# Xinglab/abPOA

Measured on AMD Instinct MI355X. Metric: read-sets/sec (consensus bit-exact) + DP Gcells/sec (roofline.dp_gcells_per_s), higher is better.
Workload: dtype int16

## Files before the change

### abpoa_amd/csrc/engine.cpp

```cpp
#include <hip/hip_runtime.h>
#include <stdio.h>
#include <stdlib.h>
#include <string.h>
#include <stdarg.h>
#include <limits.h>
#include <mutex>
#include <vector>
#include <algorithm>
#include "engine_options.h"
#include "batch_stream.h"
#include "routing.h"
#include "dir_plane.h"

namespace abpoa_hip {

static char g_err[512] = ""; static std::mutex g_err_mu;
static thread_local char g_err_copy[512] = "";
static thread_local char tl_err[512] = "";
void set_err(const char *fmt, ...) {
    va_list ap; va_start(ap, fmt); vsnprintf(tl_err, sizeof(tl_err), fmt, ap); va_end(ap);
    std::lock_guard<std::mutex> lk(g_err_mu);
    memcpy(g_err, tl_err, sizeof(g_err));
}
const char *thread_last_error() { return tl_err; }
void clear_thread_error() { tl_err[0] = 0; }
#define HIP_TRY(expr, code)                                                                          \
    do { hipError_t e_ = (expr); if (e_ != hipSuccess) {                                             \
// ... 351 lines not shown
const char *abpoa_hip_last_error(void) { std::lock_guard<std::mutex> lk(g_err_mu); memcpy(g_err_copy, g_err, sizeof(g_err)); return g_err_copy; }
void abpoa_hip_get_stats(abpoa_hip_stats_t *out) { std::lock_guard<std::mutex> lk(g.stats_mu); *out = g.stats; }
void abpoa_hip__dir_counts(long long *out) { out[0] = __atomic_exchange_n(&g_dir_counts[0], 0, __ATOMIC_RELAXED); out[1] = __atomic_exchange_n(&g_dir_counts[1], 0, __ATOMIC_RELAXED); }
void abpoa_hip__wide_plan(const abpoa_hip_scoring_t *sc, int max_qlen, int max_bits, int n_aln, int *out) {
    abpoa_hip::LdsPlan L; const int pn = max_bits == 16 ? 16 : 8; const int w = sc->wb + (int)(sc->wf * (float)max_qlen);
    abpoa_hip::make_lds_plan(sc, max_qlen, max_bits, abpoa_hip::band_cols(abpoa_hip::padded_width(max_qlen, pn), w, pn, true), n_aln, &L);
    out[0] = L.wide_on; out[1] = L.wfr_rows; out[2] = L.total_wide; out[3] = L.total_wide > 0 ? abpoa_hip::wide_workgroups_per_cu(L.total_wide) : 0;
    out[4] = L.w_phase_off; out[5] = L.wide_w_lo; out[6] = L.wide_w_hi;
}
void abpoa_hip__narrow_plan(const abpoa_hip_scoring_t *sc, int max_qlen, int max_bits, int n_aln, int *out) {
    abpoa_hip::LdsPlan L; const int pn = max_bits == 16 ? 16 : 8; const int w = sc->wb + (int)(sc->wf * (float)max_qlen);
    abpoa_hip::make_lds_plan(sc, max_qlen, max_bits, abpoa_hip::band_cols(abpoa_hip::padded_width(max_qlen, pn), w, pn, true), n_aln, &L);
    out[0] = L.fr_rows; out[1] = L.fr_cols; out[2] = L.bt_bytes_tail;
}
void abpoa_hip__row_launches(long long *out) { for (int i = 0; i < 3; ++i) out[i] = __atomic_exchange_n(&abpoa_hip::g_row_launches[i], 0, __ATOMIC_RELAXED); }
void abpoa_hip__debug_clocks(long long *out) { for (int i = 0; i < 10; ++i) { out[i] = g_dbg[i]; g_dbg[i] = 0; } }
void abpoa_hip_reset_stats(void) { std::lock_guard<std::mutex> lk(g.stats_mu); memset(&g.stats, 0, sizeof(g.stats)); }

void abpoa_hip_free_result(abpoa_hip_result_t *r) {
    if (!r) return;
    free(r->cigar);
    if (r->trace) {
        abpoa_hip_trace_t *t = r->trace;
        free(t->dp_beg); free(t->dp_end); free(t->dp_beg_sn); free(t->dp_end_sn); free(t->row_off); free(t->planes); free(t->row_max_i); free(t);
    }
    memset(r, 0, sizeof(*r));
}

static int validate(const abpoa_hip_scoring_t *sc, const abpoa_hip_problem_t *p, int idx) {
    if (p->n_rows < 3 || p->qlen < 0) { set_err("problem %d: n_rows=%d qlen=%d", idx, p->n_rows, p->qlen); return ABPOA_HIP_EINVAL; }
// ... 75 lines not shown
```

### abpoa_amd/csrc/engine_options.cpp

```cpp
#include "engine_options.h"
#include <atomic>
#include <cstdlib>
#include <cstring>
#include <mutex>
#include <string>

namespace abpoa_hip {
namespace {

struct Row { const char *name, *help; };
const Row kTable[] = {
    {"ABPOA_GPU_DEVICES", "P  device ordinals abpoa_hip_msa_batch spreads its batches over: all | 0,1,... (default: the device of abpoa_hip_init)"},
    {"ABPOA_GPU_BATCHES_PER_DEVICE", "P  batches dealt per device queue [2]"},
    {"ABPOA_HIP_STRICT", "P  1: a call that would hand any read-set to the host driver fails with ABPOA_HIP_ESTRICT"},
    {"ABPOA_HIP_VERBOSE", "P  per-pass timings, residency and fallback reasons on stderr"},
    {"ABPOA_HIP_HOSTGRAPH", "T  1: the host driver for every job"},
    {"ABPOA_HIP_NO_DEVICE_STRAND", "T  1: -s jobs on the host driver"},
    {"ABPOA_HIP_NO_DEVICE_LOCAL", "T  1: local-mode jobs on the host driver"},
    {"ABPOA_HIP_NO_DEVICE_GENERAL", "T  1: general-kernel jobs on the host driver"},
    {"ABPOA_HIP_DEVICE_GENERAL", "T  1: the general kernel for every device-resident job"},
    {"ABPOA_HIP_LOCKSTEP", "T  1: one launch per phase and round also where the all-rounds kernel would run"},
    {"ABPOA_HIP_LATE_TAIL", "T  1: the helpers of the all-rounds kernel's backtrack start after the row loop, not under it"},
    {"ABPOA_HIP_NODIR", "T  1: score-record arenas instead of direction words"},
    {"ABPOA_HIP_DIR_WIDE", "T  1 / 0: direction words for wide-band alignments always / never (default: by residency and memory)"},
    {"ABPOA_HIP_NOFAST", "T  1: no fast row loops (general kernel)"},
    {"ABPOA_HIP_NOWIDE", "T  1: no wide row loop"},
    {"ABPOA_HIP_NOXL", "T  1: no long-read form of the wide row loop"},
    {"ABPOA_HIP_LOCAL_TEAM", "T  1 / 0: the four-wavefront local row loop always / never"},
    {"ABPOA_HIP_WIDE_LO", "T  smallest band half-width that takes the wide loop [40]"},
    {"ABPOA_HIP_RING_ROWS", "T  depth of the wide loop's score ring (4 | 8 | 16)"},
    {"ABPOA_HIP_EXTRA_ROUTE_MIN", "T  ragged sets with fewer extra columns keep the narrow loop"},
    {"ABPOA_HIP_NO_RAGGED_SPLIT", "T  1: read-sets with ragged read ends stay in the batch of the uniform ones (no all-rounds kernel for such a job)"},
    {"ABPOA_HIP_RAGGED_CONCURRENT", "T  1: the ragged batch of a mixed job runs on a second queue of the device beside the uniform batch (measured: see LOG.md)"},
    {"ABPOA_HIP_PASS_SETS", "T  read-sets per pass of the device-resident driver"},
    {"ABPOA_HIP_FIRST_PASS", "T  start the node-slot ladder (3x, 4.5x, 6x, 4096x) at its second / third / fourth pass: 1 / 2 / 3 (profiling runs of one step)"},
    {"ABPOA_HIP_NO_PASS_HINT", "T  1: always start the ladder at 3x"},
    {"ABPOA_HIP_GROUPS", "T  read-set groups of the host driver"},
// ... 64 lines not shown
```

### abpoa_amd/csrc/msa_batch.cpp

```cpp
#include <algorithm>
#include <atomic>
#include <stdio.h>
#include <chrono>
#include <condition_variable>
#include <functional>
#include <memory>
#include <mutex>
#include <stdlib.h>
#include <string.h>
#include <thread>
#include <vector>
#include "engine_options.h"
#include "msa_batch.h"
#include "poa_graph.h"

#include <unordered_map>
namespace abpoa_hip {

namespace {
std::mutex g_dig_mu; std::unordered_map<uint64_t, uint64_t> g_dig;
uint64_t digest_mix64(uint64_t z) { z += 0x9E3779B97F4A7C15ull; z = (z ^ (z >> 30)) * 0xBF58476D1CE4E5B9ull; z = (z ^ (z >> 27)) * 0x94D049BB133111EBull; return z ^ (z >> 31); }
uint64_t digest_word_mix(uint64_t word, int i) { return digest_mix64(word + 0xD6E8FEB86659FD93ull * (uint64_t)(i + 1)); }
uint64_t digest_round(uint64_t before, int read_index, int n_cigar, uint64_t sum) { return (before * 0x9E3779B97F4A7C15ull) ^ (sum + digest_mix64(((uint64_t)(uint32_t)read_index
        << 32) | (uint32_t)n_cigar)); }
// ... 156 lines not shown
            if (rc) return rc;
            t2 = now_s();
            pool.run((int)active.size(), [&](int a) {
                const int s = active[a];
                if (fwd_st[a] != 0) { out[s].status = fwd_st[a]; return; }
                out[s].n_cells += fwd_cells[a];
                const uint64_t *cg = fwd_cig[a].data(); int ncg = (int)fwd_cig[a].size();
                const uint8_t *q = sets[s].seqs[k]; const int32_t *wq = weights_of(sets[s], k);
                const auto it = std::find(retry.begin(), retry.end(), a);
                if (it != retry.end()) {
                    const int t = (int)(it - retry.begin());
                    if (al->status(t) != 0) { out[s].status = al->status(t); return; }
                    out[s].n_cells += al->n_cells(t);
                    if (al->best_score(t) > fwd_score[a]) { cg = al->cigar(t); ncg = al->n_cigar(t); q = rc_seq[a].data(); wq = wq ? rc_w[a].data() : nullptr; if (out[s].is_rc) out[s].is_rc[k] = 1; }
                }
                try { graphs[s].add_alignment(q, sets[s].lens[k], cg, ncg, k, wq); } catch (...) { fail.store(1); }
            });
        } else
        pool.run((int)active.size(), [&](int a) {
            const int s = active[a];
            const int st = al->status(a);
            if (st != 0) { out[s].status = st; return; }
            out[s].n_cells += al->n_cells(a);
            if (cigar_digest_on()) cigar_digest_add(sets[s].seqs[0], sets[s].lens[0], k, al->cigar(a), al->n_cigar(a));
            try { graphs[s].add_alignment(sets[s].seqs[k], sets[s].lens[k], al->cigar(a), al->n_cigar(a), k, weights_of(sets[s], k)); } catch (...) { fail.store(1); }
        });
        if (fail.load()) return ABPOA_HIP_EINVAL;
        const double t3 = now_s();
        gt->sort_s += t1 - t0; gt->engine_s += t2 - t1; gt->fuse_s += t3 - t2; gt->rounds += 1;
    }
// ... 111 lines not shown
```

### abpoa_amd/csrc/msa_device.cpp

```cpp
#include <algorithm>
#include <atomic>
#include <chrono>
#include <limits.h>
#include <mutex>
#include <stdio.h>
#include <stdlib.h>
#include <string.h>
#include <thread>
#include <vector>
#include <hip/hip_runtime.h>
#include "engine_options.h"
#include "batch_stream.h"
#include "msa_device.h"
#include "poa_device.h"
#include "poa_graph.h"
#include "dir_plane.h"
#include "msa_batch.h"
#include "msa_device_debug.h"
#include "msa_device_plan.h"
#include "routing.h"

namespace abpoa_hip {

namespace {
#define HIP_OK(expr, code) do { hipError_t e_ = (expr); if (e_ != hipSuccess) { \
        set_err("%s failed: %s (%s:%d)", #expr, hipGetErrorString(e_), __FILE__, __LINE__); return code; } } while (0)

double now_s() { return std::chrono::duration<double>(std::chrono::steady_clock::now().time_since_epoch()).count(); }

template <typename F>
void parallel_ranges(int n_threads, int n, F fn) {
    const int T = std::max(1, std::min(n_threads, n / 64));
    if (T <= 1) { fn(0, n); return; }
    std::vector<std::thread> th; th.reserve(T - 1);
    for (int t = 0; t < T - 1; ++t) th.emplace_back(fn, (int)((int64_t)n * t / T), (int)((int64_t)n * (t + 1) / T));
// ... 45 lines not shown
    size_t o_cnode, o_ccov, o_cbase, o_isrc;
    size_t o_state, o_base, o_nin, o_nout, o_naln, o_in, o_out, o_outw, o_inx, o_outx, o_outwx, o_aln, o_nread, o_row, o_order0, o_order1, o_rid, o_mrank,
            o_msaoff, o_tout, o_toutw, o_tin, graph_bytes;
    size_t o_ticket, o_aln_desc, o_out_rec, o_rbase, o_rsd, o_rpd, o_rnid, o_rrem, o_poff, o_pred, o_bsn, o_esn, o_coff, o_rmi, o_cigar, o_scratch, o_ooff,
            o_orow, o_left, o_right, o_act, o_outfwd, o_cigfwd, o_retry, rows_bytes;
};

struct Job {
    DevicePlan pl; const abpoa_hip_readset_t *sets; int n_sets, n_threads, device, slot;
    Cache *C; Layout L; size_t dl_bytes;
    bool any_w, rest_up; int64_t split_at;
    PoaDev p; DevBatch b, b_rc, b_r;
    bool dbg_sync, use_rounds; size_t rounds_lds;
    std::vector<int64_t> msa_off;
    double t_begin, t_queue, t_done;
};

}

void release_msa_device_caches() {
    int cur = -1; (void)hipGetDevice(&cur);
    for (int s = 0; s < MSA_DEVICE_SLOTS; ++s) {
        std::lock_guard<std::mutex> lk(g_cache_mu[s]);
        Cache &C = g_cache[s];
        if (C.device < 0) continue;
        (void)hipSetDevice(C.device);
        if (C.stream) (void)hipStreamSynchronize(C.stream);
        C.release();
    }
    if (cur >= 0) (void)hipSetDevice(cur);
}

// ... 77 lines not shown
    if (need > free_b + given_back) {
        if (opt_set("ABPOA_HIP_VERBOSE")) fprintf(stderr,
                "[abpoa-hip] device %d: %d sets need %.1f GB in growing buffers (arenas %.1f GB), %.1f GB free + %.1f " "GB given back: splitting\n",
                J.device, J.n_sets, need / 1e9, pl.plane_tot / 1e9, free_b / 1e9, given_back / 1e9);
        set_err("device-resident job needs %zu more bytes, %zu free", need, free_b + given_back); return ABPOA_HIP_ENOMEM;
    }
    int rc;
    if ((rc = C.in.need_dev(L.in_dev_bytes)) || (rc = C.in.need_host(L.in_bytes)) || (rc = C.graph.need_dev(L.graph_bytes)) || (rc =
            C.graph.need_host(J.dl_bytes)) ||
        (rc = C.rows.need_dev(L.rows_bytes)) || (rc = C.planes.need_dev((size_t)pl.plane_tot))) return rc;
    const int n_ev = 4 * pl.max_reads + 8;
    while ((int)C.ev.size() < n_ev) { hipEvent_t e; HIP_OK(hipEventCreate(&e), ABPOA_HIP_ENODEV); C.ev.push_back(e); }
    return 0;
}

void stage_reads(const Job &J, int k_lo, int k_hi) {
    const DevicePlan &pl = J.pl; uint8_t *hi = J.C->in.host; const int64_t *roff = (const int64_t *)(hi + J.L.o_roff); uint8_t *rd = hi + J.L.o_reads;
    parallel_ranges(std::min(J.n_threads, 16), J.n_sets, [&](int lo, int hi_) {
        for (int s = lo; s < hi_; ++s) { const int64_t r0 = pl.ps[s].read0; const int ke = std::min(k_hi, J.sets[s].n_reads);
                for (int r = k_lo; r < ke; ++r) memcpy(rd + roff[r0 + r], J.sets[s].seqs[r], J.sets[s].lens[r]); }
    });
}

int upload_reads(Job &J) {
    const DevicePlan &pl = J.pl; Cache &C = *J.C; const Layout &L = J.L; const abpoa_hip_scoring_t *sc = &pl.sc;
    uint8_t *hi = C.in.host;
    memcpy(hi + L.o_sets, pl.ps.data(), sizeof(PoaSet) * J.n_sets);
    int64_t *roff = (int64_t *)(hi + L.o_roff); int32_t *rlen = (int32_t *)(hi + L.o_rlen); uint8_t *rd = hi + L.o_reads;
    J.split_at = 0;
    {
        int64_t at = 0;
        for (int k = 0; k < pl.max_reads; ++k) {
            if (k == 2) J.split_at = at;
            for (int s = 0; s < J.n_sets; ++s) if (k < J.sets[s].n_reads) { const int64_t ri = pl.ps[s].read0 + k; roff[ri] = at; rlen[ri] = J.sets[s].lens[k];
                    at += J.sets[s].lens[k]; }
        }
        if (pl.max_reads <= 2) J.split_at = at;
        roff[pl.tot_reads] = at;
    }
    stage_reads(J, 0, 2);
    if (J.any_w) {
        int32_t *wd = (int32_t *)(hi + L.o_wts);
        parallel_ranges(std::min(J.n_threads, 16), J.n_sets, [&](int lo, int hi_) {
            for (int s = lo; s < hi_; ++s) for (int r = 0; r < J.sets[s].n_reads; ++r) {
                int32_t *dst = wd + roff[pl.ps[s].read0 + r]; const int32_t *src = J.sets[s].weights ? J.sets[s].weights[r] : nullptr;
                if (src) memcpy(dst, src, 4 * (size_t)J.sets[s].lens[r]); else for (int j = 0; j < J.sets[s].lens[r]; ++j) dst[j] = 1;
            }
        });
    }
    memcpy(hi + L.o_mat, sc->mat, 4 * sc->m * sc->m);
    hipStream_t st = C.stream;
    if (!C.copy_stream) { HIP_OK(hipStreamCreateWithFlags(&C.copy_stream, hipStreamNonBlocking), ABPOA_HIP_ENODEV);
            HIP_OK(hipEventCreateWithFlags(&C.ev_copy, hipEventDisableTiming), ABPOA_HIP_ENODEV); }
    HIP_OK(hipMemcpyAsync(C.in.dev, hi, L.o_reads + (size_t)J.split_at, hipMemcpyHostToDevice, st), ABPOA_HIP_ELAUNCH);
    J.rest_up = J.split_at >= roff[pl.tot_reads];
    return 0;
}

void fill_poa_dev(Job &J) {
    const DevicePlan &pl = J.pl; Cache &C = *J.C; const Layout &L = J.L; const abpoa_hip_scoring_t *sc = &pl.sc; PoaDev &p = J.p; const bool gen_io = pl.gen_io();
    uint8_t *di = C.in.dev, *dg = C.graph.dev, *dr = C.rows.dev;
    memset(&p, 0, sizeof(p));
    p.n_sets = J.n_sets; p.m = sc->m; p.max_mat = sc->max_mat; p.min_mis = sc->min_mis; p.o1 = sc->gap_open1; p.e1 = sc->gap_ext1; p.o2 = sc->gap_open2;
    p.e2 = sc->gap_ext2;
    p.wb = sc->wb; p.wf = sc->wf; p.gap_mode = sc->gap_mode; p.max_qlen = pl.max_qlen;
    p.last_pass = pl.node_factor >= 6.0 ? 1 : 0;
    p.in_cap = pl.in_cap; p.out_cap = pl.out_cap;
    p.dig_on = cigar_digest_on() ? 1 : 0;
    p.aln_cap = pl.aln_cap; p.rid_words = pl.rid_words; p.order_mode = (pl.local || pl.extend) ? 1 : 0; p.banded = (sc->wb >= 0 || sc->zdrop > 0) ? 1 : 0;
    p.general = pl.general ? 1 : 0; p.msa_rows = 0; p.msa_cons = (pl.want_msa && pl.want_cons) ? 1 : 0;
// ... 76 lines not shown
        if (b_r.dir_mode && sc->gap_mode != ABPOA_HIP_LINEAR_GAP && !opt_on("ABPOA_HIP_LATE_TAIL")) {
            const int avail = (int)rounds_lds - b_r.lds.phase_off, tables = (SPEC_WK - 1) * SPEC_PM_ROWS * 4;
            const int ring = (b_r.lds.total_rows - b_r.lds.phase_off + 15) & ~15;
            int w_ = ((avail - tables) / SPEC_WK) & ~15, m_ = w_;
            if (w_ < ring) { m_ = ring; w_ = ((avail - tables - m_) / (SPEC_WK - 1)) & ~15; }
            if (w_ >= SPEC_EARLY_MIN) { b_r.lds.te_on = 1; b_r.lds.te_main = m_; b_r.lds.te_w = w_; }
        }
        const int n_cu = device_cu_count(J.device);
        if (nb < 1 || J.n_sets > nb * n_cu) use_rounds = false;
        if (opt_set("ABPOA_HIP_VERBOSE")) fprintf(stderr,
                "[abpoa-hip] all-rounds kernel: %s, %zu B dynamic + %d B static LDS per workgroup, %d workgroups per CU, " "backtrack window %d B, helpers %s (%d + 3 x %d B)\n",
                use_rounds ? "on" : "off", rounds_lds, st_lds, nb, b_r.lds.bt_bytes_tail, b_r.lds.te_on ? "under the row loop" : "after the row loop", b_r.lds.te_main, b_r.lds.te_w);
    }
}

int queue_job(Job &J, DeviceDebug &dbg) {
    const DevicePlan &pl = J.pl; Cache &C = *J.C; const Layout &L = J.L; PoaDev &p = J.p; const DevBatch &b = J.b;
    hipStream_t st = C.stream; uint8_t *hi = C.in.host, *hg = C.graph.host, *dg = C.graph.dev, *dr = C.rows.dev; int rc;
    const int64_t *roff = (const int64_t *)(hi + L.o_roff);
    auto stage = [&](const char *what, int k) { return dbg.stage(what, k); };
    if (pl.gen_io()) HIP_OK(hipMemsetAsync(dr + L.o_act, 1, (size_t)pl.node_tot, st), ABPOA_HIP_ELAUNCH);
    if (pl.amb) HIP_OK(hipMemsetAsync(dg + L.o_isrc, 0, (size_t)pl.tot_reads, st), ABPOA_HIP_ELAUNCH);
    J.t_queue = now_s();
    HIP_OK(hipEventRecord(C.ev[0], st), ABPOA_HIP_ELAUNCH);
    if (stage("upload", 0)) return ABPOA_HIP_ELAUNCH;
    HIP_OK(launch_poa_init(p, st), ABPOA_HIP_ELAUNCH);
    if (stage("init", 0)) return ABPOA_HIP_ELAUNCH;
    dbg.graph_check(0);
    HIP_OK(hipEventRecord(C.ev[1], st), ABPOA_HIP_ELAUNCH);
    for (int k = 1; k < pl.max_reads; ++k) {
        if (k == 2 && !J.rest_up) {
            stage_reads(J, 2, pl.max_reads);
            HIP_OK(hipMemcpyAsync(C.in.dev + L.o_reads + (size_t)J.split_at, hi + L.o_reads + (size_t)J.split_at, (size_t)(roff[pl.tot_reads] - J.split_at),
                    hipMemcpyHostToDevice, C.copy_stream), ABPOA_HIP_ELAUNCH);
            HIP_OK(hipEventRecord(C.ev_copy, C.copy_stream), ABPOA_HIP_ELAUNCH);
            HIP_OK(hipStreamWaitEvent(st, C.ev_copy, 0), ABPOA_HIP_ELAUNCH);
            J.rest_up = true;
        }
        if (J.use_rounds && k == 2) {
            HIP_OK(hipEventRecord(C.ev[2], st), ABPOA_HIP_ELAUNCH);
            HIP_OK(launch_poa_rounds(p, J.b_r, (int32_t *)(dr + L.o_ticket), C.in.host + L.o_rargs, J.slot, 2, J.rounds_lds, st), ABPOA_HIP_ELAUNCH);
            HIP_OK(hipEventRecord(C.ev[3], st), ABPOA_HIP_ELAUNCH);
            break;
        }
        p.round = k;
        hipEvent_t *e = C.ev.data() + 4 * k;
        if (p.order_mode) { HIP_OK(launch_poa_order(p, st), ABPOA_HIP_ELAUNCH); if (stage("row order", k)) return ABPOA_HIP_ELAUNCH; dbg.order_check(k); }
        HIP_OK(launch_poa_prepare(p, st), ABPOA_HIP_ELAUNCH);
        if (stage("prepare", k)) return ABPOA_HIP_ELAUNCH;
        dbg.prepare_check(k);
        HIP_OK(hipEventRecord(e[0], st), ABPOA_HIP_ELAUNCH);
        if (pl.general) { HIP_OK(launch_dp_general(b, st), ABPOA_HIP_ELAUNCH); HIP_OK(hipEventRecord(e[1], st), ABPOA_HIP_ELAUNCH); }
        else HIP_OK(launch_dp_fast(b, st, e[1]), ABPOA_HIP_ELAUNCH);
        if (stage("dp rows + tail", k)) return ABPOA_HIP_ELAUNCH;
        if (pl.amb) {
            HIP_OK(launch_poa_strand_check(p, st), ABPOA_HIP_ELAUNCH);
            HIP_OK(launch_dp_general(J.b_rc, st), ABPOA_HIP_ELAUNCH);
            HIP_OK(launch_poa_strand_pick(p, st), ABPOA_HIP_ELAUNCH);
            if (stage("strand retry", k)) return ABPOA_HIP_ELAUNCH;
        }
        dbg.balance_report(k, b, e[0], e[1]);
        HIP_OK(hipEventRecord(e[2], st), ABPOA_HIP_ELAUNCH);
        HIP_OK(launch_poa_fuse(p, st), ABPOA_HIP_ELAUNCH);
        if (stage("fuse", k)) return ABPOA_HIP_ELAUNCH;
        dbg.graph_check(k);
        HIP_OK(hipEventRecord(e[3], st), ABPOA_HIP_ELAUNCH);
    }
    if (pl.want_cons) { HIP_OK(launch_poa_consensus(p, st), ABPOA_HIP_ELAUNCH); if (stage("consensus", pl.max_reads)) return ABPOA_HIP_ELAUNCH; }
    if (pl.want_msa) { HIP_OK(launch_poa_msa_rank(p, st), ABPOA_HIP_ELAUNCH); if (stage("msa rank", pl.max_reads)) return ABPOA_HIP_ELAUNCH; }
    HIP_OK(hipMemcpyAsync(hg, dg, J.dl_bytes, hipMemcpyDeviceToHost, st), ABPOA_HIP_ELAUNCH);
    HIP_OK(hipStreamSynchronize(st), ABPOA_HIP_ELAUNCH);
    int64_t msa_total = 0;
    if (pl.want_msa) {
        const PoaState *hs_ = (const PoaState *)(hg + L.o_state);
        J.msa_off.resize(J.n_sets);
        for (int s = 0; s < J.n_sets; ++s) { J.msa_off[s] = msa_total; if (hs_[s].status == POA_ST_OK && hs_[s].n_nodes > 2) msa_total += (int64_t)(J.sets[s].n_reads
                + (pl.want_cons ? 1 : 0)) * std::max(0, hs_[s].msa_len); }
        if (msa_total > 0) {
            if ((rc = C.msa.need_dev((size_t)msa_total)) || (rc = C.msa.need_host((size_t)msa_total))) return rc;
            memcpy(hi + L.o_msaoff_h, J.msa_off.data(), 8 * (size_t)J.n_sets);
            HIP_OK(hipMemcpyAsync(dg + L.o_msaoff, hi + L.o_msaoff_h, 8 * (size_t)J.n_sets, hipMemcpyHostToDevice, st), ABPOA_HIP_ELAUNCH);
            p.msa_out = C.msa.dev;
            HIP_OK(launch_poa_msa_fill(p, st), ABPOA_HIP_ELAUNCH);
            if (stage("msa fill", pl.max_reads)) return ABPOA_HIP_ELAUNCH;
            HIP_OK(hipMemcpyAsync(C.msa.host, C.msa.dev, (size_t)msa_total, hipMemcpyDeviceToHost, st), ABPOA_HIP_ELAUNCH);
            HIP_OK(hipStreamSynchronize(st), ABPOA_HIP_ELAUNCH);
        }
    }
    J.t_done = now_s();
    return 0;
}

void fill_stats(const Job &J, DeviceRunStats *stats) {
    const DevicePlan &pl = J.pl; Cache &C = *J.C; const Layout &L = J.L; const PoaDev &p = J.p;
    if (opt_set("ABPOA_HIP_ORDER_PROF") && p.order_mode) {
        const PoaState *hs_ = (const PoaState *)(C.graph.host + L.o_state); double a_[4] = {0, 0, 0, 0};
        for (int s = 0; s < J.n_sets; ++s) for (int i = 0; i < 4; ++i) a_[i] += (double)hs_[s].t_phase[i];
        fprintf(stderr, "[abpoa-hip] order walk per set: %.0f single-node passes x %.0f ticks, %.0f parallel passes x %.0f ticks\n", a_[2] / J.n_sets,
                a_[2] > 0 ? a_[0] / a_[2] : 0.0, a_[3] / J.n_sets, a_[3] > 0 ? a_[1] / a_[3] : 0.0);
    }
    if (!stats) return;
    float ms = 0;
    hipEvent_t prev = C.ev[1];
    for (int k = 1; k < (J.use_rounds ? 2 : pl.max_reads); ++k) {
        hipEvent_t *e = C.ev.data() + 4 * k;
        (void)hipEventElapsedTime(&ms, prev, e[0]); stats->prepare_ms += ms;
        (void)hipEventElapsedTime(&ms, e[0], e[1]); stats->rows_ms += ms;
        (void)hipEventElapsedTime(&ms, e[1], e[2]); stats->tail_ms += ms;
        (void)hipEventElapsedTime(&ms, e[2], e[3]); stats->fuse_ms += ms;
// ... 14 lines not shown
            static const char *const ph_[4] = {"prepare", "rows", "backtrack", "fuse"};
            std::vector<double> v_((size_t)J.n_sets);
            for (int i = 0; i < 4; ++i) {
                for (int s = 0; s < J.n_sets; ++s) v_[s] = (double)hs_[s].t_phase[i];
                std::sort(v_.begin(), v_.end());
                fprintf(stderr, "[abpoa-hip] all-rounds kernel, M ticks per set, %-9s: mean %.3f  p99 %.3f  max %.3f\n", ph_[i], tp[i] / J.n_sets * 1e-6,
                        v_[(size_t)std::min<long long>(J.n_sets - 1, (long long)J.n_sets * 99 / 100)] * 1e-6, v_[(size_t)J.n_sets - 1] * 1e-6);
            }
            fprintf(stderr, "[abpoa-hip] all-rounds kernel, set totals: mean %.3f M ticks, max %.3f M ticks, max / mean %.3f\n", tall / J.n_sets * 1e-6, tmax * 1e-6,
                    tmax / (tall / J.n_sets));
        }
    }
    stats->n_rounds = pl.max_reads > 0 ? pl.max_reads - 1 : 0; stats->device_s = J.t_done - J.t_queue;
}

void collect_results(const Job &J, DeviceDebug &dbg, abpoa_hip_msa_t *out, std::vector<char> &need_fb, std::vector<SetFallback> *fallback) {
    const DevicePlan &pl = J.pl; Cache &C = *J.C; const Layout &L = J.L; const PoaDev &p = J.p; const uint8_t *hg = C.graph.host;
    const PoaState *hs = (const PoaState *)(hg + L.o_state);
    const int32_t *h_cnode = (const int32_t *)(hg + L.o_cnode), *h_ccov = (const int32_t *)(hg + L.o_ccov); const uint8_t *h_cbase = hg + L.o_cbase;
    need_fb.assign(J.n_sets, 0);
    std::vector<AlnOut> h_out;
    if (p.dig_on && J.n_sets > 0) { h_out.resize((size_t)J.n_sets);
            if (hipMemcpy(h_out.data(), p.out, sizeof(AlnOut) * (size_t)J.n_sets, hipMemcpyDeviceToHost) != hipSuccess) h_out.clear(); }
    parallel_ranges(std::min(J.n_threads, 8), J.n_sets, [&](int lo, int hi_) {
        for (int s = lo; s < hi_; ++s) {
            abpoa_hip_msa_t &o_ = out[s];
            memset(&o_, 0, sizeof(o_)); o_.n_reads = J.sets[s].n_reads;
            if (pl.amb && hs[s].status == POA_ST_OK) { o_.is_rc = (uint8_t *)calloc((size_t)std::max(1, J.sets[s].n_reads), 1);
                    if (o_.is_rc) memcpy(o_.is_rc, hg + L.o_isrc + pl.ps[s].read0, (size_t)J.sets[s].n_reads); }
            if (hs[s].status != POA_ST_OK) { need_fb[s] = 1;
                    if (J.dbg_sync) fprintf(stderr, "[poa-device] set %d falls back to the host driver: reason %d, %d nodes of %d\n", s, hs[s].reason,
                    hs[s].n_nodes, pl.ps[s].node_cap); continue; }
            o_.n_cells = hs[s].n_cells;
            if (p.dig_on && J.sets[s].n_reads > 0) cigar_digest_set(J.sets[s].seqs[0], J.sets[s].lens[0], hs[s].cigar_dig);
            if (!h_out.empty() && J.sets[s].n_reads > 1) { const AlnOut &a_ = h_out[(size_t)s];
                    const int32_t v8[8] = {a_.n_matched_bases, a_.n_aln_bases, a_.node_s, a_.node_e, a_.query_s, a_.query_e, a_.n_cigar, a_.status};
                    last_aln_set(J.sets[s].seqs[0], J.sets[s].lens[0], v8); }
            if (pl.want_cons && hs[s].n_nodes > 2) {
                const int len = hs[s].cons_len; const int64_t c0 = pl.ps[s].cons0;
                o_.cons_len = len;
                o_.cons_base = (uint8_t *)malloc(len + 1); o_.cons_cov = (int32_t *)malloc(4 * (len + 1)); o_.cons_node_id = (int32_t *)malloc(4 * (len + 1));
                memcpy(o_.cons_base, h_cbase + c0, len); memcpy(o_.cons_cov, h_ccov + c0, 4 * (size_t)len);
                memcpy(o_.cons_node_id, h_cnode + c0, 4 * (size_t)len);
            }
            if (pl.want_msa && hs[s].n_nodes > 2) {
                const int len = std::max(0, hs[s].msa_len);
                o_.msa_len = len; o_.msa_rows = J.sets[s].n_reads + (pl.want_cons ? 1 : 0);
                o_.msa_base = (uint8_t *)malloc((size_t)o_.msa_rows * (len > 0 ? len : 1));
                if (len > 0) memcpy(o_.msa_base, C.msa.host + J.msa_off[s], (size_t)o_.msa_rows * len);
            }
        }
    });
    dbg.msa_check(hs, out);
    dbg.consensus_check(hs, out);
    for (int s = 0; s < J.n_sets; ++s) if (need_fb[s]) fallback->push_back({s, host_reason_of(hs[s].reason), hs[s].reason == POA_WHY_EDGE_SLOTS});
}

void report_fallbacks(const Job &J, const std::vector<SetFallback> &fallback) {
    const PoaState *hs = (const PoaState *)(J.C->graph.host + J.L.o_state);
    if (!opt_set("ABPOA_HIP_VERBOSE") || fallback.empty()) return;
    int n[MSA_HOST_REASONS] = {0};
    int dp_scores = 0;
    for (const SetFallback &f : fallback) {
        const int r = hs[f.set].reason;
        n[f.why]++;
        if (r - POA_WHY_DP_STATUS == ABPOA_HIP_STATUS_NEED_SCORES) dp_scores++;
        if (f.why == HOST_WHY_ORDER_WALK || f.why == HOST_WHY_RANK_WALK || (f.why == HOST_WHY_OTHER && r != POA_WHY_NONE)) fprintf(stderr,
// ... 5 lines not shown
    fprintf(stderr, "[abpoa-hip] fallback reasons: node cap at init %d, pred CSR cap %d, cigar cap %d, node slots in the fuse "
            "phase %d, edge slots of a node full (redone in the last pass) %d, DP status %d, projected node growth "
            "(early exit at read 10) %d, other %d\n", n[HOST_WHY_NODES_AT_INIT], n[HOST_WHY_PRED_SLOTS], n[HOST_WHY_CIGAR_SLOTS], n[HOST_WHY_NODES_IN_FUSE],
            n[HOST_WHY_EDGE_SLOTS], n_dp, n[HOST_WHY_GROWTH], n[HOST_WHY_OTHER] + n[HOST_WHY_ORDER_WALK] + n[HOST_WHY_RANK_WALK]);
}

void finish_stats(const Job &J, const std::vector<char> &need_fb, DeviceRunStats *stats) {
    const PoaState *hs = (const PoaState *)(J.C->graph.host + J.L.o_state);
    stats->cons_s = now_s() - J.t_done; stats->total_s = now_s() - J.t_begin;
    for (int s = 0; s < J.n_sets; ++s) if (!need_fb[s]) {
        stats->n_cells += hs[s].n_cells; stats->algo_bytes += hs[s].algo_bytes; stats->n_alignments += std::max(0, J.sets[s].n_reads - 1);
        int mx = 0; for (int r = 0; r < J.sets[s].n_reads; ++r) mx = std::max(mx, J.sets[s].lens[r]);
        if ((int64_t)hs[s].n_nodes <= 2 + (int64_t)(3.0 * mx) + 1024) stats->n_fit_3x += 1;
    }
}
}

static int run_msa_device_body(const abpoa_hip_scoring_t *sc_in, int n_sets, const abpoa_hip_readset_t *sets, abpoa_hip_msa_t *out, int n_threads,
                               const DevicePass &pass, std::vector<SetFallback> *fallback, DeviceRunStats *stats, bool force_general, bool *want_general) {
    const int slot = pass.slot; int device = pass.device;
    if (slot < 0 || slot >= MSA_DEVICE_SLOTS) { set_err("bad device slot %d", slot); return ABPOA_HIP_EINVAL; }
    std::lock_guard<std::mutex> lk(g_cache_mu[slot]);
    if (device < 0) device = engine_device();
    if (device < 0) { set_err("engine not initialised"); return ABPOA_HIP_ENODEV; }
    Job J; int rc;
    J.sets = sets; J.n_sets = n_sets; J.n_threads = n_threads; J.device = device; J.slot = slot; J.C = &g_cache[slot];
    if ((rc = acquire_cache_slot(*J.C, device))) return rc;
    fallback->clear();
    if (stats) memset(stats, 0, sizeof(*stats));
    J.t_begin = now_s();
    J.pl = plan_device_job(sc_in, n_sets, sets, pass.node_factor, pass.flags, force_general);
    J.any_w = false; for (int s = 0; s < n_sets && !J.any_w; ++s) J.any_w = sets[s].weights != nullptr;
    lay_out(J.pl, n_sets, J.any_w, J.L, &J.dl_bytes);
    if ((rc = fit_device(J)) || (rc = upload_reads(J))) return rc;
    fill_poa_dev(J);
    if ((rc = fill_dev_batch(J, want_general))) return rc;
    plan_rounds(J);
    DeviceDebug dbg(&J.p, &J.pl.ps, sets, n_sets, J.pl.sc.m, J.pl.aln_cap, J.pl.max_reads, J.pl.want_msa, J.pl.amb, J.C->stream);
    if ((rc = queue_job(J, dbg))) return rc;
    fill_stats(J, stats);
    std::vector<char> need_fb;
    collect_results(J, dbg, out, need_fb, fallback);
    report_fallbacks(J, *fallback);
    if (stats) finish_stats(J, need_fb, stats);
    return ABPOA_HIP_OK;
}

int run_msa_device(const abpoa_hip_scoring_t *sc, int n_sets, const abpoa_hip_readset_t *sets, abpoa_hip_msa_t *out, int n_threads, const DevicePass &pass,
                   std::vector<SetFallback> *fallback, DeviceRunStats *stats) {
    bool want_general = false;
    const int rc = run_msa_device_body(sc, n_sets, sets, out, n_threads, pass, fallback, stats, false, &want_general);
    if (rc != ABPOA_HIP_EINVAL || !want_general) return rc;
    want_general = false;
    return run_msa_device_body(sc, n_sets, sets, out, n_threads, pass, fallback, stats, true, &want_general);
}

}
```

### abpoa_amd/csrc/msa_device.h

```cpp
#pragma once
#include <stdint.h>
#include <vector>
#include "../../include/abpoa_hip.h"
#include "device_codes.h"

namespace abpoa_hip {

struct DeviceRunStats {
    double prepare_ms, rows_ms, tail_ms, fuse_ms;
    double device_s, cons_s, total_s;
    int64_t n_cells, algo_bytes, n_alignments; int32_t n_rounds, n_fit_3x;
    double rounds_ms, rounds_rows_share, rounds_mean_over_max; int32_t rounds_launches, pad2;
    int64_t rounds_algo_bytes;
    double rounds_mticks[4];
};

bool msa_device_eligible(const abpoa_hip_scoring_t *sc, unsigned flags);
inline bool msa_device_set_is_ragged(const abpoa_hip_readset_t &S) {
    if (S.n_reads < 2) return false;
    int mx = 0, mn = 0x7fffffff;
    for (int r = 0; r < S.n_reads; ++r) { mx = S.lens[r] > mx ? S.lens[r] : mx; mn = S.lens[r] < mn ? S.lens[r] : mn; }
    const int tol = mx / 8 > 64 ? mx / 8 : 64;
    return mx - mn > tol;
}

enum HostReason : int32_t {
    HOST_WHY_OTHER = 0, HOST_WHY_NODES_AT_INIT = 1, HOST_WHY_PRED_SLOTS = 2, HOST_WHY_CIGAR_SLOTS = 3, HOST_WHY_NODES_IN_FUSE = 4, HOST_WHY_EDGE_SLOTS = 5,
    HOST_WHY_GROWTH = 6, HOST_WHY_ORDER_WALK = 7, HOST_WHY_RANK_WALK = 8, HOST_WHY_DP_ARENA = 9, HOST_WHY_DP_OTHER = 10,
    HOST_WHY_JOB = 11,
};
// ... 16 lines not shown
```

Measured before the change: 20350.

## Stage later-round reads in pieces on a worker team overlapping round 1

Read staging for rounds 2 and later now runs in the background on a persistent work team. That staging is cut into pieces of at least a few MB, and each piece is uploaded on the copy stream as soon as it is staged, instead of staging everything serially at round 2 and sending it in one copy. The host-side memcpy then overlaps with the round-1 GPU work, and the upload starts earlier. The same team also replaces parallel_ranges for result collection. Step timeline instrumentation and a cigar digest hook are added. The costs are thread-pool startup per job, a mutex and condition-variable handoff per task, and more small async copies.

```diff
diff --git a/abpoa_amd/csrc/engine.cpp b/abpoa_amd/csrc/engine.cpp
--- a/abpoa_amd/csrc/engine.cpp
+++ b/abpoa_amd/csrc/engine.cpp
@@ -11,6 +11,7 @@
 #include "batch_stream.h"
 #include "routing.h"
 #include "dir_plane.h"
+#include "msa_device.h"
 
 namespace abpoa_hip {
 
@@ -392,6 +393,7 @@
     out[0] = L.fr_rows; out[1] = L.fr_cols; out[2] = L.bt_bytes_tail;
 }
 void abpoa_hip__row_launches(long long *out) { for (int i = 0; i < 3; ++i) out[i] = __atomic_exchange_n(&abpoa_hip::g_row_launches[i], 0, __ATOMIC_RELAXED); }
+int abpoa_hip__step_timeline(double *out, int n) { return abpoa_hip::step_timeline(out, n); }
 void abpoa_hip__debug_clocks(long long *out) { for (int i = 0; i < 10; ++i) { out[i] = g_dbg[i]; g_dbg[i] = 0; } }
 void abpoa_hip_reset_stats(void) { std::lock_guard<std::mutex> lk(g.stats_mu); memset(&g.stats, 0, sizeof(g.stats)); }
 
diff --git a/abpoa_amd/csrc/engine_options.cpp b/abpoa_amd/csrc/engine_options.cpp
--- a/abpoa_amd/csrc/engine_options.cpp
+++ b/abpoa_amd/csrc/engine_options.cpp
@@ -21,6 +21,7 @@
     {"ABPOA_HIP_DEVICE_GENERAL", "T  1: the general kernel for every device-resident job"},
     {"ABPOA_HIP_LOCKSTEP", "T  1: one launch per phase and round also where the all-rounds kernel would run"},
     {"ABPOA_HIP_LATE_TAIL", "T  1: the helpers of the all-rounds kernel's backtrack start after the row loop, not under it"},
+    {"ABPOA_HIP_UPLOAD_PIECE", "T  least bytes of a piece of the later rounds' upload behind round 1 [4194304]; 0: one piece, sent when all of it is staged"},
     {"ABPOA_HIP_NODIR", "T  1: score-record arenas instead of direction words"},
     {"ABPOA_HIP_DIR_WIDE", "T  1 / 0: direction words for wide-band alignments always / never (default: by residency and memory)"},
     {"ABPOA_HIP_NOFAST", "T  1: no fast row loops (general kernel)"},
diff --git a/abpoa_amd/csrc/msa_batch.cpp b/abpoa_amd/csrc/msa_batch.cpp
--- a/abpoa_amd/csrc/msa_batch.cpp
+++ b/abpoa_amd/csrc/msa_batch.cpp
@@ -194,6 +194,7 @@
                     out[s].n_cells += al->n_cells(t);
                     if (al->best_score(t) > fwd_score[a]) { cg = al->cigar(t); ncg = al->n_cigar(t); q = rc_seq[a].data(); wq = wq ? rc_w[a].data() : nullptr; if (out[s].is_rc) out[s].is_rc[k] = 1; }
                 }
+                if (cigar_digest_on()) cigar_digest_add(sets[s].seqs[0], sets[s].lens[0], k, cg, ncg);
                 try { graphs[s].add_alignment(q, sets[s].lens[k], cg, ncg, k, wq); } catch (...) { fail.store(1); }
             });
         } else
diff --git a/abpoa_amd/csrc/msa_device.cpp b/abpoa_amd/csrc/msa_device.cpp
--- a/abpoa_amd/csrc/msa_device.cpp
+++ b/abpoa_amd/csrc/msa_device.cpp
@@ -2,6 +2,7 @@
 #include <atomic>
 #include <chrono>
 #include <limits.h>
+#include <memory>
 #include <mutex>
 #include <stdio.h>
 #include <stdlib.h>
@@ -19,6 +20,8 @@
 #include "msa_device_debug.h"
 #include "msa_device_plan.h"
 #include "routing.h"
+#include "upload_pieces.h"
+#include "work_team.h"
 
 namespace abpoa_hip {
 
@@ -94,8 +97,18 @@
     bool dbg_sync, use_rounds; size_t rounds_lds;
     std::vector<int64_t> msa_off;
     double t_begin, t_queue, t_done;
+    std::vector<int64_t> round_start; std::vector<UploadPiece> pieces; std::unique_ptr<std::atomic<int>[]> piece_left;
+    double t_entry, tl[TL_N];
+    void stamp(int i) { tl[i] = now_s() - t_entry; }
 };
-
+std::mutex g_tl_mu; double g_tl[TL_N];
+
+}
+
+int step_timeline(double *out, int n) {
+    std::lock_guard<std::mutex> lk(g_tl_mu);
+    for (int i = 0; i < n && i < TL_N; ++i) out[i] = g_tl[i];
+    return TL_N;
 }
 
 void release_msa_device_caches() {
@@ -203,31 +216,48 @@
     return 0;
 }
 
-void stage_reads(const Job &J, int k_lo, int k_hi) {
+void stage_reads(const Job &J, int k_lo, int k_hi, int s_lo, int s_hi) {
     const DevicePlan &pl = J.pl; uint8_t *hi = J.C->in.host; const int64_t *roff = (const int64_t *)(hi + J.L.o_roff); uint8_t *rd = hi + J.L.o_reads;
-    parallel_ranges(std::min(J.n_threads, 16), J.n_sets, [&](int lo, int hi_) {
-        for (int s = lo; s < hi_; ++s) { const int64_t r0 = pl.ps[s].read0; const int ke = std::min(k_hi, J.sets[s].n_reads);
-                for (int r = k_lo; r < ke; ++r) memcpy(rd + roff[r0 + r], J.sets[s].seqs[r], J.sets[s].lens[r]); }
-    });
-}
-
-int upload_reads(Job &J) {
+    for (int s = s_lo; s < s_hi; ++s) { const int64_t r0 = pl.ps[s].read0; const int ke = std::min(k_hi, J.sets[s].n_reads);
+            for (int r = k_lo; r < ke; ++r) memcpy(rd + roff[r0 + r], J.sets[s].seqs[r], J.sets[s].lens[r]); }
+}
+
+int64_t upload_piece_bytes() { const char *e = opt_env("ABPOA_HIP_UPLOAD_PIECE"); return e ? std::max(0LL, atoll(e)) : 4LL << 20; }
+
+int team_size(const Job &J) { return std::max(1, std::min(std::min(J.n_threads, 16), J.n_sets / 64)); }
+void start_team(const Job &J, WorkTeam &team) { team.start(team_size(J) - 1); }
+
+int upload_reads(Job &J, WorkTeam &team) {
     const DevicePlan &pl = J.pl; Cache &C = *J.C; const Layout &L = J.L; const abpoa_hip_scoring_t *sc = &pl.sc;
     uint8_t *hi = C.in.host;
     memcpy(hi + L.o_sets, pl.ps.data(), sizeof(PoaSet) * J.n_sets);
     int64_t *roff = (int64_t *)(hi + L.o_roff); int32_t *rlen = (int32_t *)(hi + L.o_rlen); uint8_t *rd = hi + L.o_reads;
-    J.split_at = 0;
+    J.split_at = 0; J.round_start.assign((size_t)std::max(0, pl.max_reads) + 1, 0);
     {
         int64_t at = 0;
         for (int k = 0; k < pl.max_reads; ++k) {
             if (k == 2) J.split_at = at;
+            J.round_start[k] = at;
             for (int s = 0; s < J.n_sets; ++s) if (k < J.sets[s].n_reads) { const int64_t ri = pl.ps[s].read0 + k; roff[ri] = at; rlen[ri] = J.sets[s].lens[k];
                     at += J.sets[s].lens[k]; }
         }
         if (pl.max_reads <= 2) J.split_at = at;
-        roff[pl.tot_reads] = at;
-    }
-    stage_reads(J, 0, 2);
+        roff[pl.tot_reads] = at; J.round_start[std::max(0, pl.max_reads)] = at;
+    }
+    J.rest_up = J.split_at >= roff[pl.tot_reads];
+    {
+        if (!J.rest_up) J.pieces = cut_upload_pieces(J.round_start.data(), pl.max_reads, upload_piece_bytes());
+        const int n_p = (int)J.pieces.size(), T = team_size(J);
+        J.piece_left.reset(new std::atomic<int>[(size_t)n_p + 1]);
+        for (int i = 0; i <= n_p; ++i) J.piece_left[i].store(T, std::memory_order_relaxed);
+        team.run((n_p + 1) * T, [&J, T](int t) {
+            const int i = t / T, w = t % T; const int k_lo = i ? J.pieces[(size_t)i - 1].k_lo : 0, k_hi = i ? J.pieces[(size_t)i - 1].k_hi : 2;
+            stage_reads(J, k_lo, k_hi, (int)((int64_t)J.n_sets * w / T), (int)((int64_t)J.n_sets * (w + 1) / T));
+            J.piece_left[i].fetch_sub(1, std::memory_order_acq_rel);
+        });
+        start_team(J, team);
+        team.help_until([&J] { return J.piece_left[0].load(std::memory_order_acquire) == 0; });
+    }
     if (J.any_w) {
         int32_t *wd = (int32_t *)(hi + L.o_wts);
         parallel_ranges(std::min(J.n_threads, 16), J.n_sets, [&](int lo, int hi_) {
@@ -242,7 +272,6 @@
     if (!C.copy_stream) { HIP_OK(hipStreamCreateWithFlags(&C.copy_stream, hipStreamNonBlocking), ABPOA_HIP_ENODEV);
             HIP_OK(hipEventCreateWithFlags(&C.ev_copy, hipEventDisableTiming), ABPOA_HIP_ENODEV); }
     HIP_OK(hipMemcpyAsync(C.in.dev, hi, L.o_reads + (size_t)J.split_at, hipMemcpyHostToDevice, st), ABPOA_HIP_ELAUNCH);
-    J.rest_up = J.split_at >= roff[pl.tot_reads];
     return 0;
 }
 
@@ -349,7 +378,7 @@
     }
 }
 
-int queue_job(Job &J, DeviceDebug &dbg) {
+int queue_job(Job &J, DeviceDebug &dbg, WorkTeam &team) {
     const DevicePlan &pl = J.pl; Cache &C = *J.C; const Layout &L = J.L; PoaDev &p = J.p; const DevBatch &b = J.b;
     hipStream_t st = C.stream; uint8_t *hi = C.in.host, *hg = C.graph.host, *dg = C.graph.dev, *dr = C.rows.dev; int rc;
     const int64_t *roff = (const int64_t *)(hi + L.o_roff);
@@ -364,18 +393,26 @@
     dbg.graph_check(0);
     HIP_OK(hipEventRecord(C.ev[1], st), ABPOA_HIP_ELAUNCH);
     for (int k = 1; k < pl.max_reads; ++k) {
+        if (k == 2) J.stamp(TL_ROUND1);
         if (k == 2 && !J.rest_up) {
-            stage_reads(J, 2, pl.max_reads);
-            HIP_OK(hipMemcpyAsync(C.in.dev + L.o_reads + (size_t)J.split_at, hi + L.o_reads + (size_t)J.split_at, (size_t)(roff[pl.tot_reads] - J.split_at),
-                    hipMemcpyHostToDevice, C.copy_stream), ABPOA_HIP_ELAUNCH);
+            const int n_p = (int)J.pieces.size();
+            for (int i = 0; i < n_p; ++i) {
+                team.help_until([&J, i] { return J.piece_left[i + 1].load(std::memory_order_acquire) == 0; });
+                if (i == n_p - 1) J.stamp(TL_STAGED);
+                const UploadPiece &pc = J.pieces[(size_t)i];
+                HIP_OK(hipMemcpyAsync(C.in.dev + L.o_reads + (size_t)pc.lo, hi + L.o_reads + (size_t)pc.lo, (size_t)(pc.hi - pc.lo), hipMemcpyHostToDevice,
+                        C.copy_stream), ABPOA_HIP_ELAUNCH);
+            }
             HIP_OK(hipEventRecord(C.ev_copy, C.copy_stream), ABPOA_HIP_ELAUNCH);
             HIP_OK(hipStreamWaitEvent(st, C.ev_copy, 0), ABPOA_HIP_ELAUNCH);
             J.rest_up = true;
+            J.stamp(TL_UPLOAD2);
         }
         if (J.use_rounds && k == 2) {
             HIP_OK(hipEventRecord(C.ev[2], st), ABPOA_HIP_ELAUNCH);
             HIP_OK(launch_poa_rounds(p, J.b_r, (int32_t *)(dr + L.o_ticket), C.in.host + L.o_rargs, J.slot, 2, J.rounds_lds, st), ABPOA_HIP_ELAUNCH);
             HIP_OK(hipEventRecord(C.ev[3], st), ABPOA_HIP_ELAUNCH);
+            J.stamp(TL_LAUNCHED);
             break;
         }
         p.round = k;
@@ -401,10 +438,19 @@
         dbg.graph_check(k);
         HIP_OK(hipEventRecord(e[3], st), ABPOA_HIP_ELAUNCH);
     }
+    {
+        const double t_now = now_s() - J.t_entry;
+        if (J.tl[TL_ROUND1] == 0) J.tl[TL_ROUND1] = t_now;
+        if (J.tl[TL_STAGED] == 0) J.tl[TL_STAGED] = J.tl[TL_ROUND1];
+        if (J.tl[TL_UPLOAD2] == 0) J.tl[TL_UPLOAD2] = J.tl[TL_STAGED];
+        if (J.tl[TL_LAUNCHED] == 0) J.tl[TL_LAUNCHED] = t_now;
+    }
     if (pl.want_cons) { HIP_OK(launch_poa_consensus(p, st), ABPOA_HIP_ELAUNCH); if (stage("consensus", pl.max_reads)) return ABPOA_HIP_ELAUNCH; }
     if (pl.want_msa) { HIP_OK(launch_poa_msa_rank(p, st), ABPOA_HIP_ELAUNCH); if (stage("msa rank", pl.max_reads)) return ABPOA_HIP_ELAUNCH; }
     HIP_OK(hipMemcpyAsync(hg, dg, J.dl_bytes, hipMemcpyDeviceToHost, st), ABPOA_HIP_ELAUNCH);
+    HIP_OK(hipEventRecord(C.ev[4 * pl.max_reads], st), ABPOA_HIP_ELAUNCH);
     HIP_OK(hipStreamSynchronize(st), ABPOA_HIP_ELAUNCH);
+    J.stamp(TL_SYNCED);
     int64_t msa_total = 0;
     if (pl.want_msa) {
         const PoaState *hs_ = (const PoaState *)(hg + L.o_state);
@@ -426,8 +472,14 @@
     return 0;
 }
 
-void fill_stats(const Job &J, DeviceRunStats *stats) {
+void fill_stats(Job &J, DeviceRunStats *stats) {
     const DevicePlan &pl = J.pl; Cache &C = *J.C; const Layout &L = J.L; const PoaDev &p = J.p;
+    if (J.use_rounds) {
+        float t_[4] = {0, 0, 0, 0};
+        (void)hipEventElapsedTime(&t_[0], C.ev[0], C.ev[1]); (void)hipEventElapsedTime(&t_[1], C.ev[7], C.ev[2]);
+        (void)hipEventElapsedTime(&t_[2], C.ev[2], C.ev[3]); (void)hipEventElapsedTime(&t_[3], C.ev[3], C.ev[4 * pl.max_reads]);
+        for (int i = 0; i < 4; ++i) J.tl[TL_GPU_INIT + i] = t_[i];
+    }
     if (opt_set("ABPOA_HIP_ORDER_PROF") && p.order_mode) {
         const PoaState *hs_ = (const PoaState *)(C.graph.host + L.o_state); double a_[4] = {0, 0, 0, 0};
         for (int s = 0; s < J.n_sets; ++s) for (int i = 0; i < 4; ++i) a_[i] += (double)hs_[s].t_phase[i];
@@ -472,7 +524,7 @@
     stats->n_rounds = pl.max_reads > 0 ? pl.max_reads - 1 : 0; stats->device_s = J.t_done - J.t_queue;
 }
 
-void collect_results(const Job &J, DeviceDebug &dbg, abpoa_hip_msa_t *out, std::vector<char> &need_fb, std::vector<SetFallback> *fallback) {
+void collect_results(const Job &J, DeviceDebug &dbg, WorkTeam &team, abpoa_hip_msa_t *out, std::vector<char> &need_fb, std::vector<SetFallback> *fallback) {
     const DevicePlan &pl = J.pl; Cache &C = *J.C; const Layout &L = J.L; const PoaDev &p = J.p; const uint8_t *hg = C.graph.host;
     const PoaState *hs = (const PoaState *)(hg + L.o_state);
     const int32_t *h_cnode = (const int32_t *)(hg + L.o_cnode), *h_ccov = (const int32_t *)(hg + L.o_ccov); const uint8_t *h_cbase = hg + L.o_cbase;
@@ -480,7 +532,9 @@
     std::vector<AlnOut> h_out;
     if (p.dig_on && J.n_sets > 0) { h_out.resize((size_t)J.n_sets);
             if (hipMemcpy(h_out.data(), p.out, sizeof(AlnOut) * (size_t)J.n_sets, hipMemcpyDeviceToHost) != hipSuccess) h_out.clear(); }
-    parallel_ranges(std::min(J.n_threads, 8), J.n_sets, [&](int lo, int hi_) {
+    const int T = team_size(J);
+    team.run(T, [&, T](int w) {
+        const int lo = (int)((int64_t)J.n_sets * w / T), hi_ = (int)((int64_t)J.n_sets * (w + 1) / T);
         for (int s = lo; s < hi_; ++s) {
             abpoa_hip_msa_t &o_ = out[s];
             memset(&o_, 0, sizeof(o_)); o_.n_reads = J.sets[s].n_reads;
@@ -509,6 +563,7 @@
             }
         }
     });
+    team.wait_all();
     dbg.msa_check(hs, out);
     dbg.consensus_check(hs, out);
     for (int s = 0; s < J.n_sets; ++s) if (need_fb[s]) fallback->push_back({s, host_reason_of(hs[s].reason), hs[s].reason == POA_WHY_EDGE_SLOTS});
@@ -544,11 +599,25 @@
         if ((int64_t)hs[s].n_nodes <= 2 + (int64_t)(3.0 * mx) + 1024) stats->n_fit_3x += 1;
     }
 }
+
+void report_timeline(const Job &J, DeviceRunStats *stats) {
+    const double *t = J.tl;
+    if (stats) memcpy(stats->tl, t, sizeof(J.tl));
+    { std::lock_guard<std::mutex> lk(g_tl_mu); memcpy(g_tl, t, sizeof(g_tl)); }
+    if (!opt_set("ABPOA_HIP_VERBOSE")) return;
+    fprintf(stderr, "[abpoa-hip] step timeline: sets %d rounds %d bytes %lld pieces %d | host ms: plan %.3f fit %.3f upload1 %.3f round1 %.3f staged %.3f upload2 %.3f "
+            "launched %.3f synced %.3f stats %.3f collected %.3f | gpu ms: init %.3f upload_wait %.3f rounds %.3f download %.3f\n", J.n_sets, J.pl.max_reads,
+            (long long)J.pl.tot_bases, (int)J.pieces.size(), (t[TL_PLAN] - t[TL_ENTRY]) * 1e3, (t[TL_FIT] - t[TL_PLAN]) * 1e3, (t[TL_UPLOAD1] - t[TL_FIT]) * 1e3,
+            (t[TL_ROUND1] - t[TL_UPLOAD1]) * 1e3, (t[TL_STAGED] - t[TL_ROUND1]) * 1e3, (t[TL_UPLOAD2] - t[TL_STAGED]) * 1e3, (t[TL_LAUNCHED] - t[TL_UPLOAD2]) * 1e3,
+            (t[TL_SYNCED] - t[TL_LAUNCHED]) * 1e3, (t[TL_STATS] - t[TL_SYNCED]) * 1e3, (t[TL_COLLECTED] - t[TL_STATS]) * 1e3, t[TL_GPU_INIT], t[TL_GPU_UPLOAD_WAIT],
+            t[TL_GPU_ROUNDS], t[TL_GPU_DOWNLOAD]);
+}
 }
 
 static int run_msa_device_body(const abpoa_hip_scoring_t *sc_in, int n_sets, const abpoa_hip_readset_t *sets, abpoa_hip_msa_t *out, int n_threads,
                                const DevicePass &pass, std::vector<SetFallback> *fallback, DeviceRunStats *stats, bool force_general, bool *want_general) {
     const int slot = pass.slot; int device = pass.device;
+    const double t_entry = now_s();
     if (slot < 0 || slot >= MSA_DEVICE_SLOTS) { set_err("bad device slot %d", slot); return ABPOA_HIP_EINVAL; }
     std::lock_guard<std::mutex> lk(g_cache_mu[slot]);
     if (device < 0) device = engine_device();
@@ -558,21 +627,29 @@
     if ((rc = acquire_cache_slot(*J.C, device))) return rc;
     fallback->clear();
     if (stats) memset(stats, 0, sizeof(*stats));
-    J.t_begin = now_s();
+    J.t_begin = now_s(); J.t_entry = t_entry; memset(J.tl, 0, sizeof(J.tl));
     J.pl = plan_device_job(sc_in, n_sets, sets, pass.node_factor, pass.flags, force_general);
+    J.stamp(TL_PLAN);
     J.any_w = false; for (int s = 0; s < n_sets && !J.any_w; ++s) J.any_w = sets[s].weights != nullptr;
     lay_out(J.pl, n_sets, J.any_w, J.L, &J.dl_bytes);
-    if ((rc = fit_device(J)) || (rc = upload_reads(J))) return rc;
+    if ((rc = fit_device(J))) return rc;
+    J.stamp(TL_FIT);
+    WorkTeam team;
+    if ((rc = upload_reads(J, team))) return rc;
+    J.stamp(TL_UPLOAD1);
     fill_poa_dev(J);
     if ((rc = fill_dev_batch(J, want_general))) return rc;
     plan_rounds(J);
     DeviceDebug dbg(&J.p, &J.pl.ps, sets, n_sets, J.pl.sc.m, J.pl.aln_cap, J.pl.max_reads, J.pl.want_msa, J.pl.amb, J.C->stream);
-    if ((rc = queue_job(J, dbg))) return rc;
+    if ((rc = queue_job(J, dbg, team))) return rc;
     fill_stats(J, stats);
+    J.stamp(TL_STATS);
     std::vector<char> need_fb;
-    collect_results(J, dbg, out, need_fb, fallback);
+    collect_results(J, dbg, team, out, need_fb, fallback);
+    J.stamp(TL_COLLECTED);
     report_fallbacks(J, *fallback);
     if (stats) finish_stats(J, need_fb, stats);
+    report_timeline(J, stats);
     return ABPOA_HIP_OK;
 }
 
diff --git a/abpoa_amd/csrc/msa_device.h b/abpoa_amd/csrc/msa_device.h
--- a/abpoa_amd/csrc/msa_device.h
+++ b/abpoa_amd/csrc/msa_device.h
@@ -13,7 +13,12 @@
     double rounds_ms, rounds_rows_share, rounds_mean_over_max; int32_t rounds_launches, pad2;
     int64_t rounds_algo_bytes;
     double rounds_mticks[4];
+    double tl[20];
 };
+enum StepTimeline : int { TL_ENTRY = 0, TL_PLAN, TL_FIT, TL_UPLOAD1, TL_ROUND1, TL_STAGED, TL_UPLOAD2, TL_LAUNCHED, TL_SYNCED, TL_STATS, TL_COLLECTED,
+        TL_GPU_INIT, TL_GPU_UPLOAD_WAIT, TL_GPU_ROUNDS, TL_GPU_DOWNLOAD, TL_N };
+static_assert(TL_N <= 20, "DeviceRunStats.tl");
+int step_timeline(double *out, int n);
 
 bool msa_device_eligible(const abpoa_hip_scoring_t *sc, unsigned flags);
 inline bool msa_device_set_is_ragged(const abpoa_hip_readset_t &S) {
diff --git a/abpoa_amd/csrc/upload_pieces.h b/abpoa_amd/csrc/upload_pieces.h
--- /dev/null
+++ b/abpoa_amd/csrc/upload_pieces.h
@@ -0,0 +1,23 @@
+#pragma once
+#include <stdint.h>
+#include <vector>
+
+namespace abpoa_hip {
+
+struct UploadPiece { int k_lo, k_hi; int64_t lo, hi; };
+
+inline std::vector<UploadPiece> cut_upload_pieces(const int64_t *round_start, int n_rounds, int64_t piece) {
+    std::vector<UploadPiece> v;
+    if (n_rounds <= 2) return v;
+    const int64_t total = round_start[n_rounds];
+    if (total <= round_start[2]) return v;
+    int k0 = 2;
+    for (int k = 2; k < n_rounds; ++k) {
+        const int64_t end = round_start[k + 1];
+        if (piece > 0 && end - round_start[k0] >= piece && total - end >= piece) { v.push_back({k0, k + 1, round_start[k0], end}); k0 = k + 1; }
+    }
+    v.push_back({k0, n_rounds, round_start[k0], total});
+    return v;
+}
+
+}
diff --git a/abpoa_amd/csrc/work_team.h b/abpoa_amd/csrc/work_team.h
--- /dev/null
+++ b/abpoa_amd/csrc/work_team.h
@@ -0,0 +1,63 @@
+#pragma once
+#include <condition_variable>
+#include <functional>
+#include <mutex>
+#include <thread>
+#include <vector>
+
+namespace abpoa_hip {
+
+class WorkTeam {
+public:
+    WorkTeam() = default;
+    WorkTeam(const WorkTeam &) = delete;
+    WorkTeam &operator=(const WorkTeam &) = delete;
+    ~WorkTeam() {
+        { std::lock_guard<std::mutex> lk(mu_); stop_ = true; }
+        cv_work_.notify_all();
+        for (std::thread &t : th_) if (t.joinable()) t.join();
+    }
+    void start(int n_workers) {
+        if (started_) return;
+        started_ = true;
+        th_.resize(n_workers > 0 ? (size_t)n_workers : 0);
+        if (!th_.empty()) th_[0] = std::thread([this] { work(0); });
+    }
+    int workers() const { return (int)th_.size(); }
+    void run(int n, std::function<void(int)> fn) {
+        { std::lock_guard<std::mutex> lk(mu_); fn_ = std::move(fn); n_ = n; next_ = 0; done_ = 0; }
+        cv_work_.notify_all();
+    }
+    template <typename P>
+    void help_until(P ready) {
+        std::unique_lock<std::mutex> lk(mu_);
+        while (!ready()) {
+            if (next_ < n_) { const int i = next_++; lk.unlock(); fn_(i); lk.lock(); ++done_; }
+            else if (done_ < n_) cv_done_.wait(lk);
+            else break;
+        }
+    }
+    void wait_all() { help_until([] { return false; }); }
+
+private:
+    void work(size_t me) {
+        for (size_t c = 2 * me + 1; c <= 2 * me + 2 && c < th_.size(); ++c) th_[c] = std::thread([this, c] { work(c); });
+        std::unique_lock<std::mutex> lk(mu_);
+        for (;;) {
+            cv_work_.wait(lk, [this] { return stop_ || next_ < n_; });
+            if (stop_) return;
+            const int i = next_++;
+            lk.unlock(); fn_(i); lk.lock();
+            ++done_;
+            cv_done_.notify_all();
+        }
+    }
+    std::mutex mu_;
+    std::condition_variable cv_work_, cv_done_;
+    std::function<void(int)> fn_;
+    int n_ = 0, next_ = 0, done_ = 0;
+    bool stop_ = false, started_ = false;
+    std::vector<std::thread> th_;
+};
+
+}
```

Measured after the change: 20480, median of 6. About the same (+0.7%).
